# ethz-asl/okvis

Measured on AMD Instinct MI355X. Metric: Gauss-Newton iterations/sec on 10-KF x 2-cam x 400-landmark windows (batch throughput: window-iterations/s), higher is better.
Workload: dtype f64

## Files before the change

### include/okvis_amd_ba.h

```cpp
#ifndef OKVIS_AMD_BA_H_
#define OKVIS_AMD_BA_H_

#include <stdint.h>

#ifdef __cplusplus
extern "C" {
#endif

#define OKVIS_BA_ABI_VERSION 7

#define OKVIS_BA_OK 0
#define OKVIS_BA_ERR_ARG (-1)
#define OKVIS_BA_ERR_STATE (-2)
#define OKVIS_BA_ERR_UNSUPPORTED (-3)
#define OKVIS_BA_ERR_NO_DEVICE (-4)
#define OKVIS_BA_ERR_NUMERIC (-5)
#define OKVIS_BA_HIP_ERROR_BASE 1000

#define OKVIS_BA_DIST_NONE 0
#define OKVIS_BA_DIST_RADTAN 1
#define OKVIS_BA_DIST_EQUIDISTANT 2
#define OKVIS_BA_DIST_RADTAN8 3

#define OKVIS_BA_IMU_CACHE_DOUBLES 290
// ... 186 lines not shown
#define OKVIS_BA_LIST_PAIR_OFF 5
#define OKVIS_BA_LIST_PAIR_ROLE 6
#define OKVIS_BA_LIST_LM_PIECE_BEGIN 7
#define OKVIS_BA_LIST_PAIR_PIECE 8
#define OKVIS_BA_LIST_PAIR_LIST_BEGIN 9
#define OKVIS_BA_LIST_PAIR_LIST 10
#define OKVIS_BA_LIST_TASKS 11
#define OKVIS_BA_LIST_TASK_LIST 12
#define OKVIS_BA_LIST_CHUNKS 13
#define OKVIS_BA_LIST_CHUNK_DIAG_BEGIN 14
#define OKVIS_BA_LIST_CHUNK_DIAG_OUT 15
#define OKVIS_BA_LIST_CHUNK_DESC 16
#define OKVIS_BA_LIST_PIECE_PATH 17
#define OKVIS_BA_LIST_LDL_COMP 18
#define OKVIS_BA_LIST_CHAIN 19
int okvis_ba_check_window_lists(const okvis_ba_window* w, const okvis_ba_options* opt, int32_t n_windows, int32_t which,
                                int32_t* out, int64_t capacity, int64_t* n);
#define OKVIS_BA_PATCH_POSE_PRIORS 1
#define OKVIS_BA_PATCH_SB_PRIORS 2
#define OKVIS_BA_PATCH_RELPOSE 4
#define OKVIS_BA_PATCH_MARG_PRIOR 8
typedef struct okvis_ba_patch {
  int32_t n_remove_obs;  const int32_t* remove_obs;
  int32_t n_remove_lm;   const int32_t* remove_lm;
  int32_t n_remove_pose; const int32_t* remove_pose;
  int32_t n_remove_sb;   const int32_t* remove_sb;
  int32_t n_remove_imu;  const int32_t* remove_imu;
  int32_t n_add_pose; const double* add_pose;  const uint8_t* add_pose_fixed;
  int32_t n_add_sb;   const double* add_sb;    const uint8_t* add_sb_fixed;
  int32_t n_add_lm;   const double* add_lm;
// ... 198 lines not shown
```

### okvis_amd/csrc/ba_capi.hip

```cpp
#include <hip/hip_runtime.h>

#include <algorithm>
#include <array>
#include <chrono>
#include <cstdio>
#include <cstring>
#include <map>
#include <string>
#include <type_traits>
#include <vector>

#include "../../include/okvis_amd_ba.h"
#include "ba_imu.hpp"
#include "ba_chol_tiles.hpp"
#include "ba_cov.hpp"
#include "ba_lmcov.hpp"
#include "ba_predcov.hpp"
#include "ba_linearize.hpp"
#include "ba_linearize2.hpp"
#include "ba_schur2.hpp"
#include "ba_marg.hpp"
#include "ba_marg_tiles.hpp"
#include "ba_schur.hpp"
#include "ba_solve.hpp"
// ... 275 lines not shown
  Arena A;
  A.host.swap(s->stage);
  struct GiveBack {
    StageVec& a;
    StageVec& b;
    ~GiveBack() { a.swap(b); }
  } give_back{A.host, s->stage};
  std::vector<HostWin> wins(n_windows);
  const int2* pre_where = nullptr;
  const ImuCacheD* pre_src = nullptr;
  const int n_pre = pre_launch(s, n_windows, windows, &pre_where, &pre_src);
  const bool dbg_t = debug_word().upload;
  const auto t_u0 = std::chrono::steady_clock::now();
  BatchLayout L = batch_layout(s->opt, n_windows);
  if (int rc = build_batch(windows, n_windows, s->opt, L, A, wins.data())) return rc;
  const auto t_u1 = std::chrono::steady_clock::now();
  if (A.host.size() < A.size) A.host.resize(A.size, 0);
  if (A.total() > s->arena_capacity) {
    if (s->d_arena) HIP_TRY(hipFree(s->d_arena));
    s->d_arena = nullptr;
    s->arena_capacity = 0;
    const size_t cap = A.total() + A.total() / 4;
    HIP_TRY(hipMalloc(&s->d_arena, cap));
    s->arena_capacity = cap;
  }
  s->arena_bytes = A.total();
  unsigned char* zbase = s->d_arena + A.data_bytes();
  if (A.zsize) HIP_TRY(hipMemsetAsync(zbase, 0, A.zsize, s->stream));
  HIP_TRY(hipMemcpyAsync(s->d_arena, A.host.data(), A.size, hipMemcpyHostToDevice, s->stream));
  if ((size_t)n_windows > s->wins_capacity) {
// ... 1 lines not shown
    s->d_opt = nullptr;
    s->d_wins = nullptr;
    s->d_ctrl = nullptr;
    s->wins_capacity = 0;
    HIP_TRY(hipMalloc(&s->d_opt, records_bytes((size_t)n_windows)));
    s->d_wins = reinterpret_cast<WinPtrs*>(reinterpret_cast<unsigned char*>(s->d_opt) + OPT_PAD);
    s->wins_capacity = (size_t)n_windows;
  }
  s->d_ctrl = reinterpret_cast<CtrlSlot*>(reinterpret_cast<unsigned char*>(s->d_opt) + ctrl_off((size_t)n_windows));
  std::vector<WinPtrs> ptrs(n_windows);
  for (int i = 0; i < n_windows; ++i) {
    relocate(wins[i].ptrs, s->d_arena, zbase, s->opt.debug_arrays);
    wins[i].ptrs.ctrl = (decltype(wins[i].ptrs.ctrl))(&s->d_ctrl[i].c);
    ptrs[i] = wins[i].ptrs;
  }
  const BatchMax M = batch_max(wins.data(), ptrs.data(), n_windows);
  {
    const size_t wb = sizeof(WinPtrs) * (size_t)n_windows, all = records_bytes((size_t)n_windows);
    s->stage_small.resize(all);
    std::memset(s->stage_small.data(), 0, all);
    const OptD d = make_optd(s->opt, n_windows);
    std::memcpy(s->stage_small.data(), &d, sizeof(d));
    std::memcpy(s->stage_small.data() + OPT_PAD, ptrs.data(), wb);
    HIP_TRY(hipMemcpyAsync(s->d_opt, s->stage_small.data(), all, hipMemcpyHostToDevice, s->stream));
  }
  if (n_pre > 0) {
    hipLaunchKernelGGL(imu_pre_place_kernel, dim3((unsigned)n_pre), dim3(64), 0, s->stream, s->d_wins, pre_where, pre_src);
    HIP_TRY(hipGetLastError());
  }
  for (int i = 0; i < n_windows; ++i)
    if (wins[i].h0_on_device) {
// ... 119 lines not shown
      src = at((const void*)P.task_list), width = 2;
      const Group* g = reinterpret_cast<const Group*>(at((const void*)P.groups));
      count = P.n_group ? g[P.n_group - 1].tlist_end : 0;
      break;
    }
    case OKVIS_BA_LIST_CHUNKS: src = at((const void*)P.chunks), count = 2 * (int64_t)P.n_chunk; break;
    case OKVIS_BA_LIST_CHUNK_DIAG_BEGIN: src = at((const void*)P.chunk_diag_begin), count = (int64_t)P.n_chunk * nb + 1; break;
    case OKVIS_BA_LIST_CHUNK_DIAG_OUT:
      src = at((const void*)P.chunk_diag_out);
      count = reinterpret_cast<const int*>(at((const void*)P.chunk_diag_begin))[(size_t)P.n_chunk * nb];
      break;
    case OKVIS_BA_LIST_CHUNK_DESC: src = at((const void*)P.chunk_desc), count = (int64_t)P.n_chunk * SCHUR_DESC_INTS; break;
    case OKVIS_BA_LIST_PIECE_PATH: count = 1; break;
    case OKVIS_BA_LIST_LDL_COMP: count = 1; break;
    case OKVIS_BA_LIST_CHAIN: count = 1; break;
    default: return OKVIS_BA_ERR_ARG;
  }
  *n = count;
  if (capacity < count) return OKVIS_BA_ERR_ARG;
  if (which == OKVIS_BA_LIST_PIECE_PATH) {
    out[0] = P.lin2;
  } else if (which == OKVIS_BA_LIST_LDL_COMP) {
    out[0] = (int32_t)P.ldl_comp;
  } else if (which == OKVIS_BA_LIST_CHAIN) {
    out[0] = P.chain;
  } else if (width == 4) {
    if (count) std::memcpy(out, src, 4 * (size_t)count);
  } else {
    const uint16_t* s16 = static_cast<const uint16_t*>(src);
    for (int64_t i = 0; i < count; ++i) out[i] = s16[i];
// ... 630 lines not shown
int okvis_ba_profile_iterations(okvis_ba_solver* s, int n, float* ms4) {
  if (!ms4) return OKVIS_BA_ERR_ARG;
  return profile_impl(s, n, ms4, nullptr);
}
int okvis_ba_profile_launches(okvis_ba_solver* s, int n, float* ms) {
  if (!ms) return OKVIS_BA_ERR_ARG;
  return profile_impl(s, n, nullptr, ms);
}

int okvis_ba_algorithmic_bytes(okvis_ba_solver* s, int64_t* lin, int64_t* schur, int64_t* solve, int64_t* small) {
  if (!s || !s->uploaded) return OKVIS_BA_ERR_ARG;
  int64_t a = 0, b = 0, c = 0, d = 0;
  for (auto& H : s->wins) {
    a += H.bytes_lin;
    b += H.bytes_schur;
    c += H.bytes_solve;
    d += H.bytes_small;
  }
  if (lin) *lin = a;
  if (schur) *schur = b;
  if (solve) *solve = c;
  if (small) *small = d;
  return OKVIS_BA_OK;
}

int okvis_ba_synchronize(okvis_ba_solver* s) {
  if (!s) return OKVIS_BA_ERR_ARG;
  HIP_TRY(hipSetDevice(s->device));
  HIP_TRY(hipStreamSynchronize(s->stream));
  return OKVIS_BA_OK;
// ... 12 lines not shown
```

### okvis_amd/csrc/ba_schur2.hpp

```cpp
#pragma once
#include "ba_imu.hpp"
#include "ba_schur.hpp"

namespace ba {

constexpr int SCH2_MAXT_SMALL_ROWS = 64;
typedef double sch2_v4 __attribute__((ext_vector_type(4)));

__host__ __device__ constexpr int sch2_pad16(int n) { return (n + 15) / 16 * 16; }
__host__ __device__ constexpr int sch2_nlb(int trows, int budget) {
  return 4 * ((budget / (sch2_pad16(trows + 1) + sch2_pad16(trows)) - 1) / 12);
}
__host__ __device__ constexpr int sch2_tile_doubles(int trows, int nlb) { return (sch2_pad16(trows + 1) + sch2_pad16(trows)) * (3 * nlb + 1); }
constexpr int SCH2_RING = 3, SCH2_STAGE_LM = 4, SCH2_STAGE_KP = 3 * SCH2_STAGE_LM + 1;
__host__ __device__ constexpr int sch2_ring_doubles(int trows) { return SCH2_RING * sch2_tile_doubles(trows, SCH2_STAGE_LM); }

template <int SCH2_MAXT, bool SCH2_SERIAL = (SCH2_MAXT > 3)>
__device__ __forceinline__ void schur_mfma_body(const WinPtrs* __restrict__ wins, const OptD* __restrict__ optp, int tile_rows, int final_call, int nlb,
                                                const CtrlSlot* __restrict__ ctrls, int nodec, const int bx) {
  const WinPtrs& W = wins[blockIdx.y];
  const Ctrl* ctrl = &ctrls[blockIdx.y].c;
  typedef int sch2_i4 __attribute__((ext_vector_type(4)));
  const sch2_i4 chead = *reinterpret_cast<const sch2_i4*>(ctrl);
  const int spec = __builtin_amdgcn_readfirstlane(chead.y ? 1 - chead.x : chead.x);
  const int n_tp = W.n_tile * (W.n_tile + 1) / 2;
  if (bx >= W.n_chunk * n_tp) return;

  static_assert(SCH2_SERIAL || SCH2_MAXT <= 3, "the pipelined loop serves the small tiles (one tile pair per chunk)");
  extern __shared__ __attribute__((aligned(16))) double sch_smem[];
  __shared__ double s_vinv[SCHUR_CHUNK_LM_MAX][6];
  __shared__ double s_vb[SCHUR_CHUNK_LM_MAX][3];
  __shared__ double s_diag[SCHUR_TILE_BLOCKS][36];
  __shared__ double s_yb[TILE_DIM];
  __shared__ int s_dec[2];
  __shared__ double s_lambda;
  __shared__ Ctrl s_ctrl;
  __shared__ int2 s_tb[SCH2_MAXT > 3 ? 2 * SCHUR_CHUNK_LM_MAX : 2];

  const int tid = threadIdx.x, lane = tid & 63, wave = tid >> 6;
#undef SSTAMP
#define SSTAMP(k) do { if (W.prof && tid == 0 && bx == 0 && blockIdx.y == 0) W.prof[k] = (double)clock64(); } while (0)
  SSTAMP(16);
  SchurDecisionLoads dl;
  if (!nodec) schur_decision_issue(W, ctrl, tid, dl);
  const double c_mu = nodec ? ctrl->mu : 0.0, c_radius = nodec ? ctrl->radius : 1.0;
  const OptD opt = *optp;
  const int chunk = bx / n_tp;
  const int* cd = W.chunk_desc + (size_t)chunk * SCHUR_DESC_INTS;
  const int lm_begin = cd[0], lm_end = cd[1];
  const int nl = lm_end - lm_begin;

  int tp = bx - chunk * n_tp, ti = 0;
  while (tp >= ti + 1) {
    tp -= ti + 1;
    ++ti;
  }
  const int tj = tp;
  const int nblk = W.Dp / 6, Dp = W.Dp;
  const int row0 = ti * SCHUR_TILE_BLOCKS, col0 = tj * SCHUR_TILE_BLOCKS;
  const int nrow = min(SCHUR_TILE_BLOCKS, nblk - row0), ncol = min(SCHUR_TILE_BLOCKS, nblk - col0);
  const bool diag = ti == tj;
  const int rowsA = 6 * nrow + (diag ? 1 : 0), rowsB = 6 * ncol;
  const int RT = (rowsA + 15) / 16, CT = (rowsB + 15) / 16;
// ... 4 lines not shown
  if constexpr (!SCH2_SERIAL) {
    double2* z = reinterpret_cast<double2*>(sch_smem);
    for (int i = tid; i < SCH2_RING * set_doubles / 2; i += SCHUR_THREADS) z[i] = make_double2(0.0, 0.0);
  }
  constexpr int SCH2_DI = (SCHUR_TILE_BLOCKS * 36 + SCHUR_THREADS - 1) / SCHUR_THREADS, SCH2_LL = 6;
  int d_q0[SCH2_DI], d_n[SCH2_DI], d_out[SCH2_DI][SCH2_LL];
  int r_q0 = 0, r_n = 0, r_out[SCH2_LL];
#pragma unroll
  for (int q = 0; q < SCH2_LL; ++q) r_out[q] = 0;
#pragma unroll
  for (int it = 0; it < SCH2_DI; ++it) {
    d_q0[it] = d_n[it] = 0;
#pragma unroll
    for (int q = 0; q < SCH2_LL; ++q) d_out[it][q] = 0;
  }
  if (diag) {
    const int* lb_ = W.chunk_diag_begin + (size_t)chunk * nblk + row0;
#pragma unroll
    for (int it = 0; it < SCH2_DI; ++it) {
      const int e = tid + it * SCHUR_THREADS;
      if (e < nrow * 36) {
        d_q0[it] = lb_[e / 36];
        d_n[it] = lb_[e / 36 + 1] - d_q0[it];
      }
    }
    if (tid < 6 * nrow) {
      r_q0 = lb_[tid / 6];
      r_n = lb_[tid / 6 + 1] - r_q0;
    }
#pragma unroll
    for (int it = 0; it < SCH2_DI; ++it)
// ... 13 lines not shown
  }
  constexpr int SCH2_NB = SCHUR_CHUNK_LM_MAX / 4;
  int pbv[SCH2_SERIAL ? SCH2_NB + 1 : 1];
  if constexpr (SCH2_SERIAL) {
#pragma unroll
    for (int ib = 0; ib <= SCH2_NB; ++ib) pbv[ib] = cd[2 + min(ib * (nlb / 4), SCH2_NB)];
  }
  auto pb_at = [&](int ib) {
    int r = 0;
#pragma unroll
    for (int q = 0; q <= (SCH2_SERIAL ? SCH2_NB : 0); ++q)
      if (q == ib) r = pbv[q];
    return r;
  };
  static_assert(SCH2_NB + 1 <= 64, "one descriptor entry per lane");
  const int pb_lane = SCH2_SERIAL ? 0 : cd[2 + min(lane, SCH2_NB)];
  auto pb_stage = [&](int st) { return __builtin_amdgcn_readlane(pb_lane, min(st, SCH2_NB)); };
  const int nst = (nl + SCH2_STAGE_LM - 1) / SCH2_STAGE_LM;

  const double* Wb = W.W[spec];
  double wp[18];
  int f_slot = -1, f_lb = 0;
  auto load_batch = [&](int ib) {
    if constexpr (!SCH2_SERIAL) return;
    const int pp = pb_at(ib) + tid;
    f_slot = -1;
    if (!tiled && pp < pb_at(ib + 1)) {
      const double* Wp = Wb + (size_t)pp * 18;
#pragma unroll
      for (int i = 0; i < 18; ++i) wp[i] = Wp[i];
      f_slot = W.pair_off[pp] / 6;
// ... 386 lines not shown
        tile_of(tt, I, J);
#pragma unroll
        for (int r = 0; r < 4; ++r) dn[(16 * I + (lane >> 4) + 4 * r) * DS + 16 * J + (lane & 15)] = accv[t][r];
      }
    }
    if (diag) {
#pragma unroll
      for (int it = 0; it < SCH2_DI; ++it) {
        const int e = tid + it * SCHUR_THREADS;
        if (e < nrow * 36) s_diag[e / 36][e % 36] = d_u[it];
      }
    }
    __syncthreads();
    SSTAMP(22);
    const int npairs = diag ? nrow * (nrow + 1) / 2 : nrow * ncol;
    for (int e = tid; e < npairs * 36; e += SCHUR_THREADS) {
      const int pi = e / 36, k = e - 36 * pi, ii = k / 6, jj = k - 6 * ii;
      int bi, bj;
      if (diag) {
        bi = (int)((sqrtf(8.0f * pi + 1.0f) - 1.0f) * 0.5f);
        while ((bi + 1) * (bi + 2) / 2 <= pi) ++bi;
        while (bi * (bi + 1) / 2 > pi) --bi;
        bj = pi - bi * (bi + 1) / 2;
      } else {
        bi = pi / ncol;
        bj = pi - bi * ncol;
      }
      const bool dblk = diag && bi == bj;
      const bool upper = dblk && jj > ii;
      const double yw = dn[(6 * bi + (upper ? jj : ii)) * DS + 6 * bj + (upper ? ii : jj)];
      const double u = dblk ? s_diag[bi][k] : 0.0;
      const int gbi = row0 + bi, gbj = col0 + bj;
      sp[(size_t)(gbi * (gbi + 1) / 2 + gbj) * 36 + k] = u - yw;
    }
// ... 47 lines not shown
      if (tid < 6 * nrow) {
        const int gr = row0 * 6 + tid;
        sr[gr] = s_yb[tid];
        sr[Dp + gr] = r_g;
        sr[2 * Dp + gr] = r_du;
      }
    }
  }
  SSTAMP(23);
#undef SSTAMP
}


template <int SCH2_MAXT, bool SCH2_SERIAL = (SCH2_MAXT > 3)>
__global__ __launch_bounds__(SCHUR_THREADS, SCH2_MAXT <= 3 ? 3 : 2) void schur_mfma_kernel(const WinPtrs* __restrict__ wins, const OptD* __restrict__ optp,
                                                                      int tile_rows, int final_call, int nlb, const CtrlSlot* __restrict__ ctrls, int nodec) {
  schur_mfma_body<SCH2_MAXT, SCH2_SERIAL>(wins, optp, tile_rows, final_call, nlb, ctrls, nodec, (int)blockIdx.x);
}

template <int SCH2_MAXT, bool SCH2_SERIAL = (SCH2_MAXT > 3)>
__global__ __launch_bounds__(SCHUR_THREADS, 3) void schur_ride_kernel(const WinPtrs* __restrict__ wins, const OptD* __restrict__ optp, int tile_rows,
                                                                      int final_call, int nlb, const CtrlSlot* __restrict__ ctrls, int nodec, int n_small) {
  static_assert(SCHUR_THREADS == IMU_THREADS && SCHUR_THREADS == LIN_THREADS, "one block size for both kinds of workgroup");
  if ((int)blockIdx.x < n_small) {
    extern __shared__ __attribute__((aligned(16))) double sch_smem[];
    small_body<2>(wins[blockIdx.y], 0, (int)blockIdx.x, sch_smem);
    return;
  }
  schur_mfma_body<SCH2_MAXT, SCH2_SERIAL>(wins, optp, tile_rows, final_call, nlb, ctrls, nodec, (int)blockIdx.x - n_small);
}

}
```

### okvis_amd/csrc/ba_types.hpp

```cpp
#pragma once
#include <stdint.h>

namespace ba {

constexpr int GROUP_OBS = 256;
constexpr int GROUP_LM = 64;
constexpr int GROUP_PAIRS = 512;
constexpr int LIN_THREADS = 256;
constexpr int LIN2_PIECES = 128;
constexpr int SCHUR_THREADS = 256;
constexpr int SCHUR_TILE_BLOCKS = 16;
constexpr int SCHUR_LM_BATCH = 16;
constexpr int SCHUR_CHUNK_LM_MAX = 64;
constexpr int SCHUR_DESC_INTS = 2 + SCHUR_CHUNK_LM_MAX / 4 + 1 + 1;
constexpr int SOLVE_THREADS = 1024;
constexpr int MAX_D_LDS = 174;
constexpr int MAX_D = 900;
constexpr int MAX_IMU_SAMPLES = 1 << 20;
constexpr int IMU_THREADS = 256;
constexpr int IMU_H = 0, IMU_G = 465, IMU_R = 495, IMU_COST = 510;
constexpr int IMU_LIN_STRIDE = 512;
constexpr int MAX_MARG_DIM = MAX_D;

struct ObsRec {
  uint32_t lm_cam;
  uint16_t pose;
  uint16_t ext;
  double u, v, sw;
};
// ... 216 lines not shown
```

### okvis_amd/csrc/capi_index_build.inc

```
namespace {

template <class T>
size_t put(Arena& A, const std::vector<T>& v) {
  size_t off = A.alloc(std::max<size_t>(v.size(), 1) * sizeof(T));
  if (A.host.size() < A.size) A.host.resize(A.size + A.size / 2, 0);
  if (!v.empty()) std::memcpy(A.host.data() + off, v.data(), v.size() * sizeof(T));
  else std::memset(A.host.data() + off, 0, sizeof(T));
  return off;
}
size_t put_zero(Arena& A, size_t bytes) { return A.zalloc(std::max<size_t>(bytes, 8)); }
template <class T>
size_t put_n(Arena& A, const T* p, size_t n) {
  if (!p) n = 0;
  size_t off = A.alloc(std::max<size_t>(n, 1) * sizeof(T));
  if (A.host.size() < A.size) A.host.resize(A.size + A.size / 2, 0);
  if (n) std::memcpy(A.host.data() + off, p, n * sizeof(T));
  else std::memset(A.host.data() + off, 0, sizeof(T));
  return off;
}

#define OFF(field, off) P.field = reinterpret_cast<std::remove_reference<decltype(P.field)>::type>(off)

struct BuildTimes {
  bool on = debug_word().build;
// ... 1038 lines not shown
      }
    } else
      M.Dpad_large = std::max(M.Dpad_large, ((Pi.D + 5) / 6) * 6);
    M.any_ext = M.any_ext || Pi.has_ext;
    M.group_chunks = M.group_chunks && H[i].group_chunks;
    M.spec_schur = M.spec_schur && H[i].spec_ok;
  }
  if (M.group_chunks) M.spec_schur = false;
  if (!M.group_chunks)
    for (int i = 0; i < n; ++i) P[i].fuse_fast = 0;
  if (!M.group_chunks && !M.spec_schur)
    for (int i = 0; i < n; ++i) P[i].spart_buf_stride = 0;
  return M;
}

void relocate(WinPtrs& P, unsigned char* base, unsigned char* zbase, int debug) {
  unsigned char** fields = reinterpret_cast<unsigned char**>(&P.pose[0]);
  const size_t first = offsetof(WinPtrs, pose);
  const size_t n = (offsetof(WinPtrs, marg_lin) + sizeof(void*) - first) / sizeof(void*);
  for (size_t i = 0; i < n; ++i) {
    const size_t off = reinterpret_cast<size_t>(fields[i]);
    fields[i] = (off & ARENA_ZFLAG) ? zbase + (off & ~ARENA_ZFLAG) : base + off;
  }
  if (debug != 1) {
    P.obs_r[0] = P.obs_r[1] = nullptr;
    P.S = nullptr;
    P.rhs = nullptr;
    P.Dp2 = nullptr;
  }
  if (!debug) P.prof = nullptr;
// ... 10 lines not shown
```

### okvis_amd/csrc/capi_launch.inc

```
namespace {

size_t lin_smem(bool ext, bool f32 = false) {
  const int d = f32 ? (ext ? LinCfg<true, float>::SMEM_DOUBLES : LinCfg<false, float>::SMEM_DOUBLES)
                    : (ext ? LinCfg<true, double>::SMEM_DOUBLES : LinCfg<false, double>::SMEM_DOUBLES);
  return (size_t)d * sizeof(double);
}
size_t solve_smem(int Dpad, bool large) {
  return ((large ? 0 : (size_t)ldl16_area_doubles(Dpad)) + 4 * (size_t)Dpad) * sizeof(double) + 16;
}
size_t solve_smem_chain(int chain_doubles, int Dpad) { return ((size_t)chain_doubles + 4 * (size_t)Dpad) * sizeof(double) + 16; }
int lin2_step_doubles(int max_Dp, bool fuse, bool f32) {
  const int aux = fuse ? (f32 ? Lin2Cfg<float, true>::MIN_STEP_DOUBLES : Lin2Cfg<double, true>::MIN_STEP_DOUBLES) : Lin2Cfg<double, false>::MIN_STEP_DOUBLES;
  return ((max_Dp + 1) / 2) * 2 + 8 + aux;
}
size_t lin2_smem(int max_Dp, bool fuse, bool f32, bool two_rounds = false) {
  const int fixed = two_rounds ? (f32 ? Lin2Cfg<float, false, 14>::FIXED_DOUBLES : Lin2Cfg<double, false, 14>::FIXED_DOUBLES)
                    : f32 ? (fuse ? Lin2Cfg<float, true>::FIXED_DOUBLES : Lin2Cfg<float, false>::FIXED_DOUBLES)
                          : (fuse ? Lin2Cfg<double, true>::FIXED_DOUBLES : Lin2Cfg<double, false>::FIXED_DOUBLES);
  return (size_t)(fixed + lin2_step_doubles(max_Dp, fuse, f32)) * sizeof(double);
}
size_t small_smem() { return (size_t)std::max<int>(std::max<int>(ImuLds::TOTAL, EvalLds::TOTAL), 2 * MAX_MARG_DIM) * sizeof(double); }

size_t small_eval_smem() { return (size_t)std::max<int>(EvalLds::TOTAL, 2 * MAX_MARG_DIM) * sizeof(double); }

// ... 44 lines not shown
                          &solve_kernel<false, true, true>, &solve_kernel<true, false>};
enum { SCHUR_NONE, SCHUR_VALU, SCHUR_MFMA3, SCHUR_MFMA9, SCHUR_RIDE3, SCHUR_MFMA3_SERIAL, SCHUR_RIDE3_SERIAL };
enum { SMALL_NONE, SMALL_ALL, SMALL_PREPARE };
LaunchPlan make_plan(const BatchLayout& L, const BatchMax& M, const okvis_ba_options& o, int n_windows) {
  LaunchPlan p;
  const bool f32 = o.fp32_linearize != 0;
  p.fused = M.group_chunks && f32 == L.fp32 && decision_free(o);
  p.nodec = M.spec_schur && !p.fused && decision_free(o);
  p.lin2 = L.lin2, p.split_small = L.split_small, p.graph = o.use_graph != 0;
  p.n_small = M.imu + 1;
  p.trows = std::min(TILE_DIM, M.Dp);
  if (M.schur_blocks > 0 && !p.fused) {
    const bool small_tiles = schur_small_tiles(M.Dp);
    if (!M.any_ext && schur_mfma_allowed(o) && (small_tiles || (o.tuning.flags & OKVIS_BA_TUNE_SCHUR_MFMA_LARGE))) {
      p.nlb = sch2_serial_nlb(p.trows);
      const bool serial = !small_tiles || (o.tuning.flags & OKVIS_BA_TUNE_SCHUR_SERIAL_BATCHES);
      if (!serial) p.nlb = SCH2_STAGE_LM;
      const int sm = (serial ? sch2_tile_doubles(p.trows, p.nlb) : sch2_ring_doubles(p.trows)) * (int)sizeof(double);
      p.rides = small_tiles && p.nodec && L.split_small && !(o.tuning.flags & OKVIS_BA_TUNE_NO_SMALL_RIDE);
      if (p.rides) p.schur = Launch{serial ? SCHUR_RIDE3_SERIAL : SCHUR_RIDE3, p.n_small + M.schur_blocks, std::max(sm, (int)small_eval_smem())};
      else p.schur = Launch{!small_tiles ? SCHUR_MFMA9 : serial ? SCHUR_MFMA3_SERIAL : SCHUR_MFMA3, M.schur_blocks, sm};
    } else {
      p.schur = Launch{SCHUR_VALU, M.schur_blocks, (int)(2 * SCHUR_LM_BATCH * p.trows * 3 * sizeof(double))};
    }
  }
  if (M.Dpad_small > 0)
    p.solve = Launch{(M.chain ? SOLVE_CHAIN : SOLVE_DENSE) + (M.group_chunks || M.spec_schur), 0,
                     (int)(M.chain ? solve_smem_chain(M.chain_doubles, M.Dpad_small) : solve_smem(M.Dpad_small, false))};
  if (M.Dpad_large > 0) {
    p.tiled = Launch{SOLVE_TILED, 0, (int)solve_smem(M.Dpad_large, true)};
    p.nT = (M.Dpad_large + CT_TB - 1) / CT_TB;
// ... 58 lines not shown

__global__ void delay_kernel(long long ticks) {
  const long long t0 = wall_clock64();
  while (wall_clock64() - t0 < ticks) __builtin_amdgcn_s_sleep(32);
}

struct Sub { hipStream_t st; int w0, nw, helpers; };
Sub sub(hipStream_t st, const Extent& e) { return Sub{st, e.w0, e.nw, e.helpers}; }
Sub whole(okvis_ba_solver* s) { return sub(s->stream, s->plan.whole); }

hipError_t launch_schur(okvis_ba_solver* s, Sub b, int final_call = 0) {
  const LaunchPlan& p = s->plan;
  const dim3 grid((unsigned)p.schur.gx, (unsigned)b.nw), blk(SCHUR_THREADS);
  const WinPtrs* wins = s->d_wins + b.w0;
  const CtrlSlot* ctrls = s->d_ctrl + b.w0;
  switch (p.schur.k) {
    case SCHUR_NONE: return hipSuccess;
    case SCHUR_VALU: hipLaunchKernelGGL(schur_kernel, grid, blk, p.schur.lds, b.st, wins, s->d_opt, p.trows, final_call); break;
    case SCHUR_MFMA3: hipLaunchKernelGGL(schur_mfma_kernel<3>, grid, blk, p.schur.lds, b.st, wins, s->d_opt, p.trows, final_call, p.nlb, ctrls, p.nodec); break;
    case SCHUR_MFMA9: hipLaunchKernelGGL(schur_mfma_kernel<9>, grid, blk, p.schur.lds, b.st, wins, s->d_opt, p.trows, final_call, p.nlb, ctrls, p.nodec); break;
    case SCHUR_RIDE3: hipLaunchKernelGGL(schur_ride_kernel<3>, grid, blk, p.schur.lds, b.st, wins, s->d_opt, p.trows, final_call, p.nlb, ctrls, p.nodec, p.n_small); break;
    case SCHUR_MFMA3_SERIAL: hipLaunchKernelGGL((schur_mfma_kernel<3, true>), grid, blk, p.schur.lds, b.st, wins, s->d_opt, p.trows, final_call, p.nlb, ctrls, p.nodec); break;
    case SCHUR_RIDE3_SERIAL: hipLaunchKernelGGL((schur_ride_kernel<3, true>), grid, blk, p.schur.lds, b.st, wins, s->d_opt, p.trows, final_call, p.nlb, ctrls, p.nodec, p.n_small); break;
  }
  return hipGetLastError();
}
void launch_solve_kernel(okvis_ba_solver* s, const Launch& l, dim3 grid, hipStream_t st, const WinPtrs* wins, int final_only, CtrlSlot* ctrls) {
  const SolveFn fn = SOLVE[l.k];
  hipLaunchKernelGGL(fn, grid, dim3(SOLVE_THREADS), l.lds, st, wins, s->d_opt, final_only, ctrls);
}
hipError_t launch_solve(okvis_ba_solver* s, Sub b, int final_only) {
  const LaunchPlan& p = s->plan;
  if (p.solve.k) launch_solve_kernel(s, p.solve, dim3((unsigned)b.nw, 1 + b.helpers), b.st, s->d_wins + b.w0, final_only, s->d_ctrl + b.w0);
  if (p.tiled.k) {
    launch_solve_kernel(s, p.tiled, dim3((unsigned)b.nw), b.st, s->d_wins + b.w0, final_only, s->d_ctrl + b.w0);
    if (!final_only) {
      const int nT = p.nT;
      hipLaunchKernelGGL(large_export_kernel, dim3(nT * (nT + 1) / 2, (unsigned)b.nw, CT_TILE / CT_THREADS), dim3(CT_THREADS), 0, b.st,
// ... 95 lines not shown
```

### okvis_amd/csrc/capi_solver.inc

```
namespace {

#define HIP_TRY(expr)                                              \
  do {                                                             \
    hipError_t _e = (expr);                                        \
    if (_e != hipSuccess) {                                        \
      s->last_hip_error = (int)_e;                                 \
      return OKVIS_BA_HIP_ERROR_BASE + (int)_e;                    \
    }                                                              \
  } while (0)

struct HostWin {
  int n_pose = 0, n_sb = 0, n_lm = 0, n_obs = 0, n_imu = 0, D = 0, Dp = 0, n_pair = 0, n_group = 0, n_chunk = 0;
  std::vector<int> pair_lm, pair_block;
  std::vector<int> pose_off, sb_off;
  int marg_dim = 0;
  bool h0_on_device = false;
  bool group_chunks = false;
  bool spec_ok = false;
  bool chain = false;
  WinPtrs ptrs;
  int acc = 0;
  int64_t bytes_lin = 0, bytes_schur = 0, bytes_solve = 0, bytes_small = 0;
};

// ... 48 lines not shown

struct BatchLayout {
  bool lin2 = false, chain = false;
  int chain_min = 1;
  bool fuse = false, spec = false;
  int schur_lm = 0, group_lm = 0;
  bool split_small = false;
  bool fp32 = false;
};
struct BatchMax {
  int group = 0, imu = 0, schur_blocks = 0, lm = 0, Dp = 0, chunks = 0;
  int Dpad_small = 0, Dpad_large = 0, chain_doubles = 0;
  bool any_ext = false, chain = false;
  bool group_chunks = false;
  bool spec_schur = false;
};
struct Launch {
  int k = 0, gx = 0, lds = 0;
};
struct Extent {
  int w0 = 0, nw = 0, helpers = 0;
  bool operator==(const Extent& o) const { return w0 == o.w0 && nw == o.nw && helpers == o.helpers; }
};
struct PlanFixed {
  int lin2 = 0, split_small = 0, fused = 0, nodec = 0, rides = 0, graph = 0;
  Launch schur; int trows = 0, nlb = 0, n_small = 0;
  Launch solve, tiled; int nT = 0;
  Launch small_init, small_iter, lin; int lin_n_small = 0, sd = 0;
  Launch take_back; int budget = 0;
  Extent whole; int one_helpers = 0;
};
struct LaunchPlan : PlanFixed {
  std::vector<Extent> subs;
  bool operator==(const LaunchPlan& o) const {
    return std::memcmp(static_cast<const PlanFixed*>(this), static_cast<const PlanFixed*>(&o), sizeof(PlanFixed)) == 0 && subs == o.subs;
  }
};

}

struct okvis_ba_solver {
  int device = 0;
  hipStream_t stream = nullptr;
  std::vector<hipStream_t> sub_streams;
  std::vector<hipEvent_t> sub_events;
  hipEvent_t ev0 = nullptr, ev1 = nullptr, ev_fork = nullptr;
  okvis_ba_options opt;
  OptD* d_opt = nullptr;
  unsigned char* d_arena = nullptr;
  size_t arena_bytes = 0, arena_capacity = 0, wins_capacity = 0;
  WinPtrs* d_wins = nullptr;
  CtrlSlot* d_ctrl = nullptr;
  StageVec stage_dl;
  StageVec stage, stage_small;
  std::vector<HostWin> wins;
  bool uploaded = false, begun = false;
  BatchLayout layout;
  BatchMax max;
  LaunchPlan plan;
  LaunchPlan graph_plan;
  std::vector<const void*> graph_addr;
  unsigned char* h_ctrl_stage = nullptr;
  unsigned char* d_ctrl_stage = nullptr;
  size_t ctrl_stage_bytes = 0;
  bool patchable = false;
  std::vector<WindowStore> mirrors;
  WindowStore mirror_edit;
// ... 88 lines not shown
  d.marg_mode = 0;
  d.dogleg = o.strategy == OKVIS_BA_STRATEGY_DOGLEG;
  d.jacobi_scaling = o.jacobi_scaling != 0;
  d.max_invalid = o.max_consecutive_invalid_steps > 0 ? o.max_consecutive_invalid_steps : 5;
  d.helper_polls = (o.reserved0 & 16) ? 0 : 1 << 22;
  return d;
}

void destroy_graphs(okvis_ba_solver* s) {
  for (auto& kv : s->graphs) (void)hipGraphExecDestroy(kv.second);
  s->graphs.clear();
  for (auto& kv : s->sub_graphs) (void)hipGraphExecDestroy(kv.second);
  s->sub_graphs.clear();
}
void keep_graphs(okvis_ba_solver* s) {
  std::vector<const void*> addr = {s->d_wins, s->d_opt, s->d_ctrl};
  for (auto st : s->sub_streams) addr.push_back(st);
  if (s->plan == s->graph_plan && addr == s->graph_addr) return;
  destroy_graphs(s);
  s->graph_plan = s->plan;
  s->graph_addr.swap(addr);
}

}
```

### okvis_amd/solver.py

```python
from __future__ import annotations

import ctypes as C
from typing import Sequence

import numpy as np

from . import _lib
from .window import LimitsC, OptionsC, SummaryC, Window, WindowC, default_options

ARR = dict(POSE=0, SB=1, LM=2, OBS_RESIDUAL=3, LM_V=4, LM_B=5, LM_HQ=6, PAIR_W=7, REDUCED_S=8,
           REDUCED_RHS=9, STEP=10, LM_QUALITY=11, GRADIENT=12, IMU_RESIDUAL=13, HPP=14, DAMPING=15, IMU_SB_REF=16, IMU_LIN=17, PROF=99, IMU_REDO_COUNT=98, CTRL=97, SLOTS=96)
_dp = C.POINTER(C.c_double)


def limits() -> dict:
    lim = LimitsC()
    _lib.lib().okvis_ba_get_limits(C.byref(lim))
    return {n: getattr(lim, n) for n, _ in lim._fields_}


def check_window(window: Window, options: OptionsC | None = None) -> dict:
    window.validate()
    wc, keep = window.as_c()
    st = (C.c_int64 * 8)()
    _lib.check(_lib.lib().okvis_ba_check_window(C.byref(wc), C.byref(options) if options is not None else None, st),
               "check_window")
    del keep
    return dict(D=st[0], Dp=st[1], n_pair=st[2], n_group=st[3], n_chunk=st[4], n_task=st[5], gpart=st[6],
                arena_bytes=st[7])


INDEX_LISTS = ("groups", "lm_obs_begin", "lm_pair_begin", "pair_lm", "pair_block", "pair_off", "pair_role", "lm_piece_begin",
               "pair_piece", "pair_list_begin", "pair_list", "tasks", "task_list", "chunks", "chunk_diag_begin", "chunk_diag_out",
               "chunk_desc", "piece_path", "ldl_comp", "chain")


def index_lists(window: Window, options: OptionsC | None = None, n_windows: int = 1) -> dict:
    wc, keep = window.as_c()
    L = _lib.lib()
    po = C.byref(options) if options is not None else None
    out = {}
    for which, name in enumerate(INDEX_LISTS):
        n = C.c_int64()
        rc = L.okvis_ba_check_window_lists(C.byref(wc), po, n_windows, which, None, 0, C.byref(n))
        if rc != 0 and not (rc == -1 and n.value > 0):
            _lib.check(rc, "check_window_lists")
        a = np.zeros(max(n.value, 1), np.int32)
        if n.value:
            _lib.check(L.okvis_ba_check_window_lists(C.byref(wc), po, n_windows, which, a.ctypes.data_as(C.POINTER(C.c_int32)), n.value,
                                                     C.byref(n)), "check_window_lists")
        out[name] = a[:n.value]
    del keep
    out["groups"] = out["groups"].reshape(-1, 16)
    out["tasks"] = out["tasks"].reshape(-1, 6)
    out["chunks"] = out["chunks"].reshape(-1, 2)
    out["piece_path"] = int(out["piece_path"][0])
    out["ldl_comp"] = int(out["ldl_comp"][0]) & 0xFFFFFFFF
    out["chain"] = int(out["chain"][0])
    return out


class WindowStore:

    def __init__(self, window: Window):
        self._L = _lib.lib()
        self._h = C.c_void_p()
        wc, keep = window.as_c()
        _lib.check(self._L.okvis_ba_store_create(C.byref(wc), C.byref(self._h)), "store_create")
        del keep

# ... 375 lines not shown
```

Measured before the change: 540,500.

## Pack per-chunk Schur index lists into contiguous launch records

```diff
diff --git a/include/okvis_amd_ba.h b/include/okvis_amd_ba.h
--- a/include/okvis_amd_ba.h
+++ b/include/okvis_amd_ba.h
@@ -224,6 +224,7 @@
 #define OKVIS_BA_LIST_PIECE_PATH 17
 #define OKVIS_BA_LIST_LDL_COMP 18
 #define OKVIS_BA_LIST_CHAIN 19
+#define OKVIS_BA_LIST_CHUNK_RECS 20
 int okvis_ba_check_window_lists(const okvis_ba_window* w, const okvis_ba_options* opt, int32_t n_windows, int32_t which,
                                 int32_t* out, int64_t capacity, int64_t* n);
 #define OKVIS_BA_PATCH_POSE_PRIORS 1
diff --git a/okvis_amd/csrc/ba_capi.hip b/okvis_amd/csrc/ba_capi.hip
--- a/okvis_amd/csrc/ba_capi.hip
+++ b/okvis_amd/csrc/ba_capi.hip
@@ -313,6 +313,8 @@
   const auto t_u0 = std::chrono::steady_clock::now();
   BatchLayout L = batch_layout(s->opt, n_windows);
   if (int rc = build_batch(windows, n_windows, s->opt, L, A, wins.data())) return rc;
+  size_t rec_off = 0;
+  const int rec_stride = build_chunk_records(A, wins.data(), n_windows, &rec_off);
   const auto t_u1 = std::chrono::steady_clock::now();
   if (A.host.size() < A.size) A.host.resize(A.size, 0);
   if (A.total() > s->arena_capacity) {
@@ -344,7 +346,9 @@
     wins[i].ptrs.ctrl = (decltype(wins[i].ptrs.ctrl))(&s->d_ctrl[i].c);
     ptrs[i] = wins[i].ptrs;
   }
-  const BatchMax M = batch_max(wins.data(), ptrs.data(), n_windows);
+  BatchMax M = batch_max(wins.data(), ptrs.data(), n_windows);
+  M.rec_stride = rec_stride;
+  s->d_recs = rec_stride ? reinterpret_cast<const int*>(s->d_arena + rec_off) : nullptr;
   {
     const size_t wb = sizeof(WinPtrs) * (size_t)n_windows, all = records_bytes((size_t)n_windows);
     s->stage_small.resize(all);
@@ -494,6 +498,12 @@
     case OKVIS_BA_LIST_PIECE_PATH: count = 1; break;
     case OKVIS_BA_LIST_LDL_COMP: count = 1; break;
     case OKVIS_BA_LIST_CHAIN: count = 1; break;
+    case OKVIS_BA_LIST_CHUNK_RECS: {
+      size_t off = 0;
+      const int stride = build_chunk_records(A, &H, 1, &off);
+      src = A.host.data() + off, count = (int64_t)stride * SCHUR_REC_INTS;
+      break;
+    }
     default: return OKVIS_BA_ERR_ARG;
   }
   *n = count;
@@ -1154,6 +1164,7 @@
   for (auto& H : s->wins) {
     a += H.bytes_lin;
     b += H.bytes_schur;
+    if (s->plan.rec_stride) b += (int64_t)H.n_chunk * SCHUR_REC_INTS * (int64_t)sizeof(int);
     c += H.bytes_solve;
     d += H.bytes_small;
   }
diff --git a/okvis_amd/csrc/ba_schur2.hpp b/okvis_amd/csrc/ba_schur2.hpp
--- a/okvis_amd/csrc/ba_schur2.hpp
+++ b/okvis_amd/csrc/ba_schur2.hpp
@@ -17,11 +17,28 @@
 
 template <int SCH2_MAXT, bool SCH2_SERIAL = (SCH2_MAXT > 3)>
 __device__ __forceinline__ void schur_mfma_body(const WinPtrs* __restrict__ wins, const OptD* __restrict__ optp, int tile_rows, int final_call, int nlb,
-                                                const CtrlSlot* __restrict__ ctrls, int nodec, const int bx) {
+                                                const CtrlSlot* __restrict__ ctrls, int nodec, const int bx, const int* __restrict__ recs,
+                                                int rec_stride) {
   const WinPtrs& W = wins[blockIdx.y];
   const Ctrl* ctrl = &ctrls[blockIdx.y].c;
   typedef int sch2_i4 __attribute__((ext_vector_type(4)));
   const sch2_i4 chead = *reinterpret_cast<const sch2_i4*>(ctrl);
+  const int* rec = SCH2_SERIAL ? nullptr : recs + ((size_t)blockIdx.y * rec_stride + bx) * SCHUR_REC_INTS;
+  constexpr int SCH2_RI = SCH2_SERIAL ? 1 : (SCH2_MAXT_SMALL_ROWS / 6 * 36 + SCHUR_THREADS - 1) / SCHUR_THREADS;
+  sch2_i4 rec_d[SCH2_RI][2], rec_r[2];
+  int rec_pb = 0;
+  if constexpr (!SCH2_SERIAL) {
+    static_assert(SCH2_MAXT_SMALL_ROWS / 6 <= SCHUR_REC_BLOCKS, "every pose block of a small tile has its entry in the record");
+    const int lane_ = threadIdx.x & 63;
+    rec_pb = rec[2 + min(lane_, SCHUR_CHUNK_LM_MAX / 4)];
+#pragma unroll
+    for (int it = 0; it < SCH2_RI; ++it) {
+      const sch2_i4* le = reinterpret_cast<const sch2_i4*>(rec + SCHUR_REC_LISTS + 8 * min(((int)threadIdx.x + it * SCHUR_THREADS) / 36, SCHUR_REC_BLOCKS - 1));
+      rec_d[it][0] = le[0], rec_d[it][1] = le[1];
+    }
+    const sch2_i4* le = reinterpret_cast<const sch2_i4*>(rec + SCHUR_REC_LISTS + 8 * min((int)threadIdx.x / 6, SCHUR_REC_BLOCKS - 1));
+    rec_r[0] = le[0], rec_r[1] = le[1];
+  }
   const int spec = __builtin_amdgcn_readfirstlane(chead.y ? 1 - chead.x : chead.x);
   const int n_tp = W.n_tile * (W.n_tile + 1) / 2;
   if (bx >= W.n_chunk * n_tp) return;
@@ -46,7 +63,7 @@
   const double c_mu = nodec ? ctrl->mu : 0.0, c_radius = nodec ? ctrl->radius : 1.0;
   const OptD opt = *optp;
   const int chunk = bx / n_tp;
-  const int* cd = W.chunk_desc + (size_t)chunk * SCHUR_DESC_INTS;
+  const int* cd = SCH2_SERIAL ? W.chunk_desc + (size_t)chunk * SCHUR_DESC_INTS : rec;
   const int lm_begin = cd[0], lm_end = cd[1];
   const int nl = lm_end - lm_begin;
 
@@ -81,7 +98,17 @@
 #pragma unroll
     for (int q = 0; q < SCH2_LL; ++q) d_out[it][q] = 0;
   }
-  if (diag) {
+  if constexpr (!SCH2_SERIAL) {
+    static_assert(SCH2_LL == SCHUR_REC_LL, "list heads of the launch record");
+#pragma unroll
+    for (int it = 0; it < SCH2_RI; ++it) {
+      d_q0[it] = rec_d[it][0].x, d_n[it] = rec_d[it][0].y;
+      d_out[it][0] = rec_d[it][0].z, d_out[it][1] = rec_d[it][0].w;
+      d_out[it][2] = rec_d[it][1].x, d_out[it][3] = rec_d[it][1].y, d_out[it][4] = rec_d[it][1].z, d_out[it][5] = rec_d[it][1].w;
+    }
+    r_q0 = rec_r[0].x, r_n = rec_r[0].y;
+    r_out[0] = rec_r[0].z, r_out[1] = rec_r[0].w, r_out[2] = rec_r[1].x, r_out[3] = rec_r[1].y, r_out[4] = rec_r[1].z, r_out[5] = rec_r[1].w;
+  } else if (diag) {
     const int* lb_ = W.chunk_diag_begin + (size_t)chunk * nblk + row0;
 #pragma unroll
     for (int it = 0; it < SCH2_DI; ++it) {
@@ -125,7 +152,7 @@
     return r;
   };
   static_assert(SCH2_NB + 1 <= 64, "one descriptor entry per lane");
-  const int pb_lane = SCH2_SERIAL ? 0 : cd[2 + min(lane, SCH2_NB)];
+  const int pb_lane = SCH2_SERIAL ? 0 : rec_pb;
   auto pb_stage = [&](int st) { return __builtin_amdgcn_readlane(pb_lane, min(st, SCH2_NB)); };
   const int nst = (nl + SCH2_STAGE_LM - 1) / SCH2_STAGE_LM;
 
@@ -542,10 +569,20 @@
     __syncthreads();
     SSTAMP(22);
     const int npairs = diag ? nrow * (nrow + 1) / 2 : nrow * ncol;
+    int pi_ = tid / 36, k_ = tid - 36 * pi_, bi_ = 0, bj_ = pi_;
+    while (bj_ > bi_) bj_ -= ++bi_;
     for (int e = tid; e < npairs * 36; e += SCHUR_THREADS) {
-      const int pi = e / 36, k = e - 36 * pi, ii = k / 6, jj = k - 6 * ii;
+      const int pi = SCH2_SERIAL ? e / 36 : pi_, k = SCH2_SERIAL ? e - 36 * pi : k_, ii = k / 6, jj = k - 6 * ii;
       int bi, bj;
-      if (diag) {
+      if constexpr (!SCH2_SERIAL) {
+        bi = diag ? bi_ : pi / ncol;
+        bj = diag ? bj_ : pi - bi * ncol;
+        const int wrap = k_ + SCHUR_THREADS % 36 >= 36;
+        k_ += SCHUR_THREADS % 36 - 36 * wrap;
+        pi_ += SCHUR_THREADS / 36 + wrap;
+        bj_ += SCHUR_THREADS / 36 + wrap;
+        while (bj_ > bi_) bj_ -= ++bi_;
+      } else if (diag) {
         bi = (int)((sqrtf(8.0f * pi + 1.0f) - 1.0f) * 0.5f);
         while ((bi + 1) * (bi + 2) / 2 <= pi) ++bi;
         while (bi * (bi + 1) / 2 > pi) --bi;
@@ -623,20 +660,22 @@
 
 template <int SCH2_MAXT, bool SCH2_SERIAL = (SCH2_MAXT > 3)>
 __global__ __launch_bounds__(SCHUR_THREADS, SCH2_MAXT <= 3 ? 3 : 2) void schur_mfma_kernel(const WinPtrs* __restrict__ wins, const OptD* __restrict__ optp,
-                                                                      int tile_rows, int final_call, int nlb, const CtrlSlot* __restrict__ ctrls, int nodec) {
-  schur_mfma_body<SCH2_MAXT, SCH2_SERIAL>(wins, optp, tile_rows, final_call, nlb, ctrls, nodec, (int)blockIdx.x);
+                                                                      int tile_rows, int final_call, int nlb, const CtrlSlot* __restrict__ ctrls, int nodec,
+                                                                      const int* __restrict__ recs, int rec_stride) {
+  schur_mfma_body<SCH2_MAXT, SCH2_SERIAL>(wins, optp, tile_rows, final_call, nlb, ctrls, nodec, (int)blockIdx.x, recs, rec_stride);
 }
 
 template <int SCH2_MAXT, bool SCH2_SERIAL = (SCH2_MAXT > 3)>
 __global__ __launch_bounds__(SCHUR_THREADS, 3) void schur_ride_kernel(const WinPtrs* __restrict__ wins, const OptD* __restrict__ optp, int tile_rows,
-                                                                      int final_call, int nlb, const CtrlSlot* __restrict__ ctrls, int nodec, int n_small) {
+                                                                      int final_call, int nlb, const CtrlSlot* __restrict__ ctrls, int nodec, int n_small,
+                                                                      const int* __restrict__ recs, int rec_stride) {
   static_assert(SCHUR_THREADS == IMU_THREADS && SCHUR_THREADS == LIN_THREADS, "one block size for both kinds of workgroup");
   if ((int)blockIdx.x < n_small) {
     extern __shared__ __attribute__((aligned(16))) double sch_smem[];
     small_body<2>(wins[blockIdx.y], 0, (int)blockIdx.x, sch_smem);
     return;
   }
-  schur_mfma_body<SCH2_MAXT, SCH2_SERIAL>(wins, optp, tile_rows, final_call, nlb, ctrls, nodec, (int)blockIdx.x - n_small);
+  schur_mfma_body<SCH2_MAXT, SCH2_SERIAL>(wins, optp, tile_rows, final_call, nlb, ctrls, nodec, (int)blockIdx.x - n_small, recs, rec_stride);
 }
 
 }
diff --git a/okvis_amd/csrc/ba_types.hpp b/okvis_amd/csrc/ba_types.hpp
--- a/okvis_amd/csrc/ba_types.hpp
+++ b/okvis_amd/csrc/ba_types.hpp
@@ -13,6 +13,8 @@
 constexpr int SCHUR_LM_BATCH = 16;
 constexpr int SCHUR_CHUNK_LM_MAX = 64;
 constexpr int SCHUR_DESC_INTS = 2 + SCHUR_CHUNK_LM_MAX / 4 + 1 + 1;
+constexpr int SCHUR_REC_INTS = 128, SCHUR_REC_LISTS = 32, SCHUR_REC_LL = 6, SCHUR_REC_BLOCKS = (SCHUR_REC_INTS - SCHUR_REC_LISTS) / 8;
+static_assert(SCHUR_DESC_INTS <= SCHUR_REC_LISTS && SCHUR_REC_LL + 2 == 8, "layout of the chunk launch record");
 constexpr int SOLVE_THREADS = 1024;
 constexpr int MAX_D_LDS = 174;
 constexpr int MAX_D = 900;
diff --git a/okvis_amd/csrc/capi_index_build.inc b/okvis_amd/csrc/capi_index_build.inc
--- a/okvis_amd/csrc/capi_index_build.inc
+++ b/okvis_amd/csrc/capi_index_build.inc
@@ -1076,6 +1076,37 @@
   return M;
 }
 
+int build_chunk_records(Arena& A, const HostWin* H, int n, size_t* off) {
+  int stride = 0;
+  for (int i = 0; i < n; ++i) {
+    const WinPtrs& P = H[i].ptrs;
+    if (P.has_ext || !schur_small_tiles(P.Dp) || P.Dp / 6 > SCHUR_REC_BLOCKS) return 0;
+    stride = std::max(stride, P.n_chunk);
+  }
+  if (stride == 0) return 0;
+  const size_t bytes = (size_t)n * stride * SCHUR_REC_INTS * sizeof(int);
+  *off = A.alloc(bytes);
+  if (A.host.size() < A.size) A.host.resize(A.size, 0);
+  std::memset(A.host.data() + *off, 0, bytes);
+  for (int i = 0; i < n; ++i) {
+    const WinPtrs& P = H[i].ptrs;
+    auto list = [&](const void* field) { return reinterpret_cast<const int*>(A.host.data() + reinterpret_cast<size_t>(field)); };
+    const int *desc = list((const void*)P.chunk_desc), *begin = list((const void*)P.chunk_diag_begin), *out = list((const void*)P.chunk_diag_out);
+    const int nb = P.Dp / 6;
+    for (int c = 0; c < P.n_chunk; ++c) {
+      int* r = reinterpret_cast<int*>(A.host.data() + *off) + ((size_t)i * stride + c) * SCHUR_REC_INTS;
+      std::memcpy(r, desc + (size_t)c * SCHUR_DESC_INTS, SCHUR_DESC_INTS * sizeof(int));
+      for (int b = 0; b < nb; ++b) {
+        int* e = r + SCHUR_REC_LISTS + 8 * b;
+        const int q0 = begin[(size_t)c * nb + b], nq = begin[(size_t)c * nb + b + 1] - q0;
+        e[0] = q0, e[1] = nq;
+        for (int q = 0; q < std::min(nq, SCHUR_REC_LL); ++q) e[2 + q] = out[q0 + q];
+      }
+    }
+  }
+  return stride;
+}
+
 void relocate(WinPtrs& P, unsigned char* base, unsigned char* zbase, int debug) {
   unsigned char** fields = reinterpret_cast<unsigned char**>(&P.pose[0]);
   const size_t first = offsetof(WinPtrs, pose);
diff --git a/okvis_amd/csrc/capi_launch.inc b/okvis_amd/csrc/capi_launch.inc
--- a/okvis_amd/csrc/capi_launch.inc
+++ b/okvis_amd/csrc/capi_launch.inc
@@ -82,7 +82,8 @@
     const bool small_tiles = schur_small_tiles(M.Dp);
     if (!M.any_ext && schur_mfma_allowed(o) && (small_tiles || (o.tuning.flags & OKVIS_BA_TUNE_SCHUR_MFMA_LARGE))) {
       p.nlb = sch2_serial_nlb(p.trows);
-      const bool serial = !small_tiles || (o.tuning.flags & OKVIS_BA_TUNE_SCHUR_SERIAL_BATCHES);
+      const bool serial = !small_tiles || M.rec_stride == 0 || (o.tuning.flags & OKVIS_BA_TUNE_SCHUR_SERIAL_BATCHES);
+      p.rec_stride = serial ? 0 : M.rec_stride;
       if (!serial) p.nlb = SCH2_STAGE_LM;
       const int sm = (serial ? sch2_tile_doubles(p.trows, p.nlb) : sch2_ring_doubles(p.trows)) * (int)sizeof(double);
       p.rides = small_tiles && p.nodec && L.split_small && !(o.tuning.flags & OKVIS_BA_TUNE_NO_SMALL_RIDE);
@@ -171,14 +172,15 @@
   const dim3 grid((unsigned)p.schur.gx, (unsigned)b.nw), blk(SCHUR_THREADS);
   const WinPtrs* wins = s->d_wins + b.w0;
   const CtrlSlot* ctrls = s->d_ctrl + b.w0;
+  const int* recs = p.rec_stride ? s->d_recs + (size_t)b.w0 * p.rec_stride * SCHUR_REC_INTS : nullptr;
   switch (p.schur.k) {
     case SCHUR_NONE: return hipSuccess;
     case SCHUR_VALU: hipLaunchKernelGGL(schur_kernel, grid, blk, p.schur.lds, b.st, wins, s->d_opt, p.trows, final_call); break;
-    case SCHUR_MFMA3: hipLaunchKernelGGL(schur_mfma_kernel<3>, grid, blk, p.schur.lds, b.st, wins, s->d_opt, p.trows, final_call, p.nlb, ctrls, p.nodec); break;
-    case SCHUR_MFMA9: hipLaunchKernelGGL(schur_mfma_kernel<9>, grid, blk, p.schur.lds, b.st, wins, s->d_opt, p.trows, final_call, p.nlb, ctrls, p.nodec); break;
-    case SCHUR_RIDE3: hipLaunchKernelGGL(schur_ride_kernel<3>, grid, blk, p.schur.lds, b.st, wins, s->d_opt, p.trows, final_call, p.nlb, ctrls, p.nodec, p.n_small); break;
-    case SCHUR_MFMA3_SERIAL: hipLaunchKernelGGL((schur_mfma_kernel<3, true>), grid, blk, p.schur.lds, b.st, wins, s->d_opt, p.trows, final_call, p.nlb, ctrls, p.nodec); break;
-    case SCHUR_RIDE3_SERIAL: hipLaunchKernelGGL((schur_ride_kernel<3, true>), grid, blk, p.schur.lds, b.st, wins, s->d_opt, p.trows, final_call, p.nlb, ctrls, p.nodec, p.n_small); break;
+    case SCHUR_MFMA3: hipLaunchKernelGGL(schur_mfma_kernel<3>, grid, blk, p.schur.lds, b.st, wins, s->d_opt, p.trows, final_call, p.nlb, ctrls, p.nodec, recs, p.rec_stride); break;
+    case SCHUR_MFMA9: hipLaunchKernelGGL(schur_mfma_kernel<9>, grid, blk, p.schur.lds, b.st, wins, s->d_opt, p.trows, final_call, p.nlb, ctrls, p.nodec, recs, p.rec_stride); break;
+    case SCHUR_RIDE3: hipLaunchKernelGGL(schur_ride_kernel<3>, grid, blk, p.schur.lds, b.st, wins, s->d_opt, p.trows, final_call, p.nlb, ctrls, p.nodec, p.n_small, recs, p.rec_stride); break;
+    case SCHUR_MFMA3_SERIAL: hipLaunchKernelGGL((schur_mfma_kernel<3, true>), grid, blk, p.schur.lds, b.st, wins, s->d_opt, p.trows, final_call, p.nlb, ctrls, p.nodec, recs, p.rec_stride); break;
+    case SCHUR_RIDE3_SERIAL: hipLaunchKernelGGL((schur_ride_kernel<3, true>), grid, blk, p.schur.lds, b.st, wins, s->d_opt, p.trows, final_call, p.nlb, ctrls, p.nodec, p.n_small, recs, p.rec_stride); break;
   }
   return hipGetLastError();
 }
diff --git a/okvis_amd/csrc/capi_solver.inc b/okvis_amd/csrc/capi_solver.inc
--- a/okvis_amd/csrc/capi_solver.inc
+++ b/okvis_amd/csrc/capi_solver.inc
@@ -86,6 +86,7 @@
   bool any_ext = false, chain = false;
   bool group_chunks = false;
   bool spec_schur = false;
+  int rec_stride = 0;
 };
 struct Launch {
   int k = 0, gx = 0, lds = 0;
@@ -96,7 +97,7 @@
 };
 struct PlanFixed {
   int lin2 = 0, split_small = 0, fused = 0, nodec = 0, rides = 0, graph = 0;
-  Launch schur; int trows = 0, nlb = 0, n_small = 0;
+  Launch schur; int trows = 0, nlb = 0, n_small = 0, rec_stride = 0;
   Launch solve, tiled; int nT = 0;
   Launch small_init, small_iter, lin; int lin_n_small = 0, sd = 0;
   Launch take_back; int budget = 0;
@@ -123,6 +124,7 @@
   size_t arena_bytes = 0, arena_capacity = 0, wins_capacity = 0;
   WinPtrs* d_wins = nullptr;
   CtrlSlot* d_ctrl = nullptr;
+  const int* d_recs = nullptr;
   StageVec stage_dl;
   StageVec stage, stage_small;
   std::vector<HostWin> wins;
@@ -241,7 +243,7 @@
   s->sub_graphs.clear();
 }
 void keep_graphs(okvis_ba_solver* s) {
-  std::vector<const void*> addr = {s->d_wins, s->d_opt, s->d_ctrl};
+  std::vector<const void*> addr = {s->d_wins, s->d_opt, s->d_ctrl, s->d_recs};
   for (auto st : s->sub_streams) addr.push_back(st);
   if (s->plan == s->graph_plan && addr == s->graph_addr) return;
   destroy_graphs(s);
diff --git a/okvis_amd/solver.py b/okvis_amd/solver.py
--- a/okvis_amd/solver.py
+++ b/okvis_amd/solver.py
@@ -32,7 +32,7 @@
 
 INDEX_LISTS = ("groups", "lm_obs_begin", "lm_pair_begin", "pair_lm", "pair_block", "pair_off", "pair_role", "lm_piece_begin",
                "pair_piece", "pair_list_begin", "pair_list", "tasks", "task_list", "chunks", "chunk_diag_begin", "chunk_diag_out",
-               "chunk_desc", "piece_path", "ldl_comp", "chain")
+               "chunk_desc", "piece_path", "ldl_comp", "chain", "chunk_recs")
 
 
 def index_lists(window: Window, options: OptionsC | None = None, n_windows: int = 1) -> dict:
@@ -54,6 +54,7 @@
     out["groups"] = out["groups"].reshape(-1, 16)
     out["tasks"] = out["tasks"].reshape(-1, 6)
     out["chunks"] = out["chunks"].reshape(-1, 2)
+    out["chunk_recs"] = out["chunk_recs"].reshape(-1, 128)
     out["piece_path"] = int(out["piece_path"][0])
     out["ldl_comp"] = int(out["ldl_comp"][0]) & 0xFFFFFFFF
     out["chain"] = int(out["chain"][0])
```

Result: faster. 548,300 (median of 6 runs) (+1.4%).
